# KyungMinJin/OTPose

Measured on AMD Instinct MI355X. Metric: frames/sec at 384x288, 5-frame window, batch 16; heatmap max-abs delta vs ref, higher is better.
Workload: dtype f32 storage+accumulate / f16x3 split products; 1 GPU; BASELINE configs[1]: batch 16 x 5-frame x 384x288, HRNet-W48 + DCN warp + ConvVideoTransformer, fp32 forward (eval), seeded synthetic weights; clips_per_gpu=16, parallelism=dp1, outputs_finite=True

## Files before the change

include/otpose_hip.h:

```cpp
#ifndef OTPOSE_HIP_H
#define OTPOSE_HIP_H

#include <stddef.h>

#ifdef __cplusplus
extern "C" {
#endif

#define OTP_OK 0
#define OTP_ERR_BAD_ARG (-1)
#define OTP_ERR_UNSUPPORTED (-2)
#define OTP_ERR_LAUNCH (-3)
#define OTP_ERR_WORKSPACE (-4)

#define OTP_DTYPE_F32 0
#define OTP_DTYPE_F16 1
#define OTP_DTYPE_BF16 2
#define OTP_DTYPE_F64 3
#define OTP_DTYPE_I64 4

#define OTP_ACT_NONE 0
#define OTP_ACT_RELU 1
#define OTP_ACT_GELU 2

// ... 160 lines not shown
                          size_t workspace_bytes, int B, int Cin, int J, int H, int W, const int* dilations, int ND, float alpha,
                          void* stream);

int otp_glue_total(const void* rough, void* total, void* squeezed, void* inter, void* flow_in, const void* pe,
                   int B, int J, int HW, void* stream);
int otp_glue_stack(const void* rough, const void* margin, const void* squeezed, const void* inter,
                   const void* ctx, const void* pe1, const void* pe2, void* x1, void* x2, void* prev_b,
                   int B, int J, int HW, void* stream);

int otp_glue_total_n(const void* rough, void* total, void* squeezed, void* inter, void* flow_in, const void* pe,
                     int B, int J, int HW, int F, void* stream);
int otp_glue_stack_n(const void* rough, const void* margin, const void* squeezed, const void* inter,
                     const void* ctx, const void* pe1, const void* pe2, void* x1, void* x2, void* prev_b,
                     int B, int J, int HW, int F, void* stream);

int otp_ln_channel(const void* x, const void* gamma, const void* beta, void* y, void* pool,
                   int B, int C, int T, float eps, void* stream);
int otp_dwconv_ln3(const void* x, const void* dwq, const void* dwk, const void* dwv,
                   const void* gq, const void* bq, const void* gk, const void* bk, const void* gv, const void* bv,
                   void* q, void* k, void* v, int B, int C, int T, int stride, float eps, void* stream);
size_t otp_chan_attn_workspace(int B, int C, int T, int n_head);
int otp_chan_attn(const void* q, const void* k, const void* v, void* out, void* workspace, size_t workspace_bytes,
                  int B, int C, int T, int n_head, float scale, void* stream);
int otp_upsample_linear(const void* x, void* out, int B, int C, int T, int f, int out_ctot, int out_coff, void* stream);

int otp_mlp_fused_supported(int C, int HID, int T);
size_t otp_mlp_fused_weight_bytes(int C, int HID);
int otp_mlp_fused_pack(const void* w1, const void* b1, const void* w2, void* packed, int C, int HID, void* stream);
int otp_mlp_fused(const void* x, const void* packed, const void* scale, const void* shift, const void* res, void* out,
                  int B, int C, int HID, int T, void* stream);
int otp_ln_mlp_fused(const void* y, const void* ln_gamma, const void* ln_beta, float ln_eps, const void* packed,
                     const void* scale, const void* shift, void* out, int B, int C, int HID, int T, void* stream);

int otp_dense_x3_supported(int C, int T);
size_t otp_dense_x3_weight_bytes(int C);
int otp_dense_x3_pack(const void* w, const void* scale, const void* shift, void* packed, int C, void* stream);
int otp_dense_x3(const void* const* x, const void* const* packed, const void* const* res, void* const* out, int nprob, int B,
                 int C, int T, void* stream);
int otp_dense_x3_pack_bf16p(const void* w, const void* scale, const void* shift, void* packed, int C, void* stream);
int otp_dense_x3_bf16p(const void* const* x, const void* const* packed, const void* const* res, void* const* out, int nprob, int B,
                 int C, int T, void* stream);
int otp_qkv_front_x3(const void* x, const void* table, const void* packed_q, const void* packed_k, const void* packed_v,
                     void* q, void* k, void* v, int B, int C, int T, float eps, void* stream);

int otp_stem_conv_x3_supported(int B, int F, int H, int W, int Cout);
size_t otp_stem_conv_x3_weight_bytes(int Cout);
int otp_stem_conv_x3_pack(const void* w, const void* scale, const void* shift, void* packed, int Cout, void* stream);
int otp_stem_conv_x3(const void* in, const void* packed, void* out, int B, int F, int H, int W, int Cout, void* stream);

int otp_pointwise_x3_supported(int Cin, int Cout, int T);
size_t otp_pointwise_x3_weight_bytes(int Cin, int Cout);
int otp_pointwise_x3_pack(const void* w, const void* scale, const void* shift, void* packed, int Cin, int Cout, void* stream);
int otp_pointwise_x3(const void* x, const void* packed, const void* res, void* out, int B, int Cin, int Cout, int T, int x_ctot,
                     int x_coff, int res_ctot, int res_coff, int out_ctot, int out_coff, int relu, void* stream);
int otp_pointwise_x3_s8_supported(int Cin, int Cout, int T);
size_t otp_pointwise_x3_s8_weight_bytes(int Cin, int Cout);
int otp_pointwise_x3_s8_pack(const void* w, const void* scale, const void* shift, void* packed, int Cin, int Cout, void* stream);
int otp_pointwise_x3_s8(const void* x, const void* packed, void* out_s8, int B, int Cin, int Cout, int T, int x_ctot, int x_coff,
                        int relu, void* stream);
int otp_pointwise_x3_s8_res(const void* x, const void* packed, const void* res, void* out_s8, int B, int Cin, int Cout, int T,
                            int x_ctot, int x_coff, int r_ctot, int r_coff, int relu, void* stream);
int otp_pointwise_x3_pair_supported(int Cin, int Cmid, int Cout2, int T);
size_t otp_pointwise_x3_pair_weight_bytes(int Cin, int Cmid, int Cout2);
int otp_pointwise_x3_pair_pack(const void* w1, const void* scale1, const void* shift1, const void* w2, const void* scale2,
                               const void* shift2, void* packed, int Cin, int Cmid, int Cout2, void* stream);
int otp_pointwise_x3_pair(const void* x, const void* packed, const void* res, void* out, void* out_s8, int B, int Cin, int Cmid,
                          int Cout2, int T, int x_ctot, int x_coff, int res_ctot, int res_coff, int out_ctot, int out_coff,
                          int relu1, int relu2, void* stream);

int otp_mlp_x3_supported(int C, int HID, int T);
size_t otp_mlp_x3_weight_bytes(int C, int HID);
int otp_mlp_x3_pack(const void* w1, const void* b1, const void* w2, void* packed, int C, int HID, void* stream);
int otp_mlp_x3(const void* x, const void* packed, const void* scale, const void* shift, const void* res, void* out, int B,
               int C, int HID, int T, void* stream);
int otp_ln_mlp_x3(const void* y, const void* ln_gamma, const void* ln_beta, float ln_eps, const void* packed,
                  const void* scale, const void* shift, void* out, int B, int C, int HID, int T, void* stream);

int otp_flow_block_supported(int C, int hidden, int T);
size_t otp_flow_front_param_floats(int C);
size_t otp_flow_back_param_floats(int C, int hidden);
int otp_flow_front(const void* x, const void* params, void* q, void* k, void* v, int B, int C, int T, float eps, void* stream);
int otp_flow_back(const void* x, const void* att, const void* params, void* out, int B, int C, int hidden, int T, float eps,
                  void* stream);

int otp_dense_cc_supported(int C, int T);
size_t otp_dense_cc_weight_bytes(int C);
int otp_dense_cc_pack(const void* w, const void* scale, const void* shift, void* packed, int C, void* stream);
int otp_dense_cc(const void* const* x, const void* const* packed, const void* const* res, void* const* out, int nprob,
                 int B, int C, int T, void* stream);

size_t otp_qkv_front_table_bytes(int C);
int otp_qkv_front_pack_table(const void* dwq, const void* dwk, const void* dwv, const void* gq, const void* bq,
                             const void* gk, const void* bk, const void* gv, const void* bv, void* table, int C,
                             void* stream);
int otp_qkv_front(const void* x, const void* table, const void* packed_q, const void* packed_k, const void* packed_v,
                  void* q, void* k, void* v, int B, int C, int T, float eps, void* stream);

int otp_upsample_add(const void* low, const void* res, void* out, int N, int C, int Hl, int Wl, int f, int relu,
                     int low_ctot, int low_coff, int res_ctot, int res_coff, int out_ctot, int out_coff, void* stream);
int otp_upsample_add_multi(const void* const* lows, const int* factors, int nlow, const void* res, void* out, int N, int C,
                           int Hh, int Wh, int relu, int res_ctot, int res_coff, int out_ctot, int out_coff, void* stream);

int otp_chan_attn_set_split(int on);
int otp_chan_attn_splits(int BH, int T);
int otp_chan_attn_scores(const void* a, const void* b, void* slabs, int BH, int hs, int T, void* stream);
int otp_chan_attn_apply(const void* v, const void* M, void* out, int BH, int hs, int T, void* stream);
int otp_chan_attn_scores_bf16p(const void* a, const void* b, void* slabs, int BH, int hs, int T, void* stream);
int otp_chan_attn_apply_bf16p(const void* v, const void* M, void* out, int BH, int hs, int T, void* stream);
int otp_transpose_scale(const void* in, void* out, int batches, int R, int Cc, float scale, void* stream);
int otp_softmax_backward(const void* slabs, const void* P, void* dS, void* dST, void* PT, int BH, int hs, int NS,
                         void* stream);
int otp_ln_channel_backward(const void* x, const void* grad_y, const void* gamma, void* grad_x, void* dy_xhat, int B, int C,
                            int T, float eps, void* stream);
size_t otp_ln_channel_backward_workspace(int B, int C, int T);
int otp_ln_channel_backward_params(const void* x, const void* grad_y, const void* gamma, void* grad_x, void* grad_gamma,
                                   void* grad_beta, void* workspace, size_t workspace_bytes, int B, int C, int T, float eps,
                                   void* stream);
int otp_dwconv3_forward(const void* x, const void* w, void* y, int B, int C, int T, int stride, void* stream);
int otp_dwconv3_backward(const void* x, const void* w, const void* grad_y, void* grad_x, void* grad_w, int B, int C, int T,
                         int stride, void* stream);
int otp_gelu_forward(const void* x, void* y, size_t n, void* stream);
int otp_gelu_backward(const void* x, const void* grad_y, void* grad_x, size_t n, void* stream);
int otp_maxpool3s2_forward(const void* x, void* y, int rows, int T, void* stream);
int otp_maxpool3s2_backward(const void* x, const void* grad_y, void* grad_x, int rows, int T, void* stream);
int otp_upsample_linear_backward(const void* grad_out, void* grad_x, int B, int C, int T, int f, int out_ctot, int out_coff,
                                 void* stream);

int otp_upsample_add_backward(const void* grad_out, const void* out_relu, void* grad_res, void* grad_low, int planes, int Hl,
                              int Wl, int f, void* stream);

int otp_axpby(const void* x, void* y, float alpha, float beta, size_t n, void* stream);

int otp_heatmap_decode(const void* heatmaps, void* preds, void* maxvals, const void* center, const void* scale,
                       int N, int J, int H, int W, int refine, void* stream);

int otp_heatmap_flip_decode(const void* heatmaps, const int* perm, void* merged, void* preds, void* maxvals,
                            const void* center, const void* scale, int B, int J, int H, int W, int shift, void* stream);
int otp_clip_mirror_pair(const void* x, void* out, int B, int C, int H, int W, void* stream);

int otp_pck_accuracy(const void* pred_coords, const void* target_coords, void* acc, void* cnt, int N, int J, int H, int W,
                     float thr, void* stream);

size_t otp_grad_sumsq_scratch(void);
int otp_grad_sumsq(const void* grad, size_t n, void* acc_f64, void* stream);
int otp_adamw_step(void* param, const void* grad, void* exp_avg, void* exp_avg_sq, size_t n, float lr, float beta1,
                   float beta2, float eps, float weight_decay, int step, const void* gradnorm_sq_f64, float max_norm,
                   void* stream);
int otp_sgd_step(void* param, const void* grad, void* momentum_buf, size_t n, float lr, float momentum, float dampening,
                 float weight_decay, int nesterov, int first_step, const void* gradnorm_sq_f64, float max_norm, void* stream);

int otp_ema_update(void* ema, const void* src, size_t n, float decay, float one_minus_decay, void* stream);
size_t otp_ema_job_bytes(void);
int otp_ema_job(void* ema, const void* src, size_t count, int dtype, const void* prev_job_host, void* job_host);
int otp_ema_update_table(const void* jobs_device, int n_jobs, float decay, float one_minus_decay, void* stream);

int otp_frames_u8_to_clip(const void* frames_u8, void* out, int B, int F, int H, int W, float mean_r, float mean_g,
                          float mean_b, float std_r, float std_g, float std_b, void* stream);

int otp_crop_clips_u8(const void* pool_u8, int S, int Hp, int Wp, const void* frame_idx, const void* M, const void* flip,
                      void* out, int B, int F, int H, int W, float mean_r, float mean_g, float mean_b, float std_r,
                      float std_g, float std_b, void* stream);
int otp_crop_clips_blur_u8(const void* pool_u8, int S, int Hp, int Wp, const void* frame_idx, const void* M,
                           const void* flip, void* out, int B, int F, int H, int W, float mean_r, float mean_g,
                           float mean_b, float std_r, float std_g, float std_b, const void* blur, const void* blur_on,
                           void* stream);
int otp_crop_clips_pair_u8(const void* pool_u8, int S, int Hp, int Wp, const void* frame_idx, const void* M, void* out,
// ... 122 lines not shown
```

otpose_amd/csrc/flowenc.hip:

```cpp
#include "common.h"

namespace {

template <int C>
__device__ __forceinline__ void fe_layer_norm(float (&v)[C], const float* __restrict__ g, const float* __restrict__ b, float eps) {
    float s = 0.f;
#pragma unroll
    for (int c = 0; c < C; ++c) s += v[c];
    const float mu = s * (1.f / C);
    float q = 0.f;
#pragma unroll
    for (int c = 0; c < C; ++c) {
        v[c] -= mu;
        q += v[c] * v[c];
    }
    const float rs = 1.f / sqrtf(q * (1.f / C) + eps);
#pragma unroll
    for (int c = 0; c < C; ++c) v[c] = v[c] * rs * g[c] + b[c];
}

template <int C>
constexpr int fe_front_floats() { return 2 * C + 3 * (3 * C + 2 * C + C * C + C); }
template <int C>
constexpr int fe_back_floats(int H) { return C * C + C + 2 * C + H * C + H + H * C + C; }

template <int C>
__global__ __launch_bounds__(192) void flow_front_kernel(const float* __restrict__ x, const float* __restrict__ prm,
                                                         float* __restrict__ q, float* __restrict__ k, float* __restrict__ v,
                                                         int T, float eps) {
    const int t = blockIdx.x * 64 + (threadIdx.x & 63);
    const int br = __builtin_amdgcn_readfirstlane(threadIdx.x >> 6);
    if (t >= T) return;
    const size_t base = (size_t)blockIdx.y * C * T + t;
    float n[3][C];
#pragma unroll
    for (int s = 0; s < 3; ++s) {
        const int tt = t - 1 + s;
        const bool ok = tt >= 0 && tt < T;
#pragma unroll
        for (int c = 0; c < C; ++c) n[s][c] = ok ? x[base + (size_t)c * T + (s - 1)] : 0.f;
        fe_layer_norm<C>(n[s], prm, prm + C, eps);
        if (!ok) {
#pragma unroll
            for (int c = 0; c < C; ++c) n[s][c] = 0.f;
        }
    }
    float* out = br == 0 ? q : (br == 1 ? k : v);
    const float* p = prm + 2 * C + br * (3 * C + 2 * C + C * C + C);
    float d[C];
#pragma unroll
    for (int c = 0; c < C; ++c) d[c] = p[c * 3] * n[0][c] + p[c * 3 + 1] * n[1][c] + p[c * 3 + 2] * n[2][c];
    fe_layer_norm<C>(d, p + 3 * C, p + 4 * C, eps);
    const float* W = p + 5 * C;
    const float* bias = W + C * C;
#pragma unroll
    for (int o = 0; o < C; ++o) {
        float a = bias[o];
#pragma unroll
        for (int c = 0; c < C; ++c) a = fmaf(W[o * C + c], d[c], a);
        out[base + (size_t)o * T] = a;
    }
}

template <int C>
__global__ __launch_bounds__(256) void flow_back_kernel(const float* __restrict__ x, const float* __restrict__ att,
                                                        const float* __restrict__ prm, float* __restrict__ out, int H, int T,
                                                        float eps) {
    __shared__ float part[3][C][64];
    const int lane = threadIdx.x & 63;
    const int wave = __builtin_amdgcn_readfirstlane(threadIdx.x >> 6);
    const int t = blockIdx.x * 64 + lane;
    const bool live = t < T;
    const size_t base = (size_t)blockIdx.y * C * T + (live ? t : 0);
    float a[C], y[C];
#pragma unroll
    for (int c = 0; c < C; ++c) {
        a[c] = att[base + (size_t)c * T];
        y[c] = x[base + (size_t)c * T];
    }
    const float* Wp = prm;
    const float* bp = Wp + C * C;
#pragma unroll
    for (int o = 0; o < C; ++o) {
        float s = bp[o];
#pragma unroll
        for (int c = 0; c < C; ++c) s = fmaf(Wp[o * C + c], a[c], s);
        y[o] += s;
    }
    float nn[C];
#pragma unroll
    for (int c = 0; c < C; ++c) nn[c] = y[c];
    fe_layer_norm<C>(nn, bp + C, bp + 2 * C, eps);
    const float* W1 = bp + 3 * C;
    const float* b1 = W1 + (size_t)H * C;
    const float* W2t = b1 + H;
    const float* b2 = W2t + (size_t)H * C;
    float acc[C];
#pragma unroll
    for (int o = 0; o < C; ++o) acc[o] = 0.f;
#pragma unroll 2
    for (int m = wave; m < H; m += 4) {
        float h = b1[m];
#pragma unroll
        for (int c = 0; c < C; ++c) h = fmaf(W1[m * C + c], nn[c], h);
        h = otp_gelu_erf(h);
#pragma unroll
        for (int o = 0; o < C; ++o) acc[o] = fmaf(W2t[m * C + o], h, acc[o]);
    }
    if (wave > 0) {
#pragma unroll
        for (int o = 0; o < C; ++o) part[wave - 1][o][lane] = acc[o];
    }
    __syncthreads();
    if (wave == 0 && live) {
#pragma unroll
        for (int o = 0; o < C; ++o)
            out[base + (size_t)o * T] = y[o] + b2[o] + ((acc[o] + part[0][o][lane]) + (part[1][o][lane] + part[2][o][lane]));
    }
}

}

extern "C" int otp_flow_block_supported(int C, int hidden, int T) { return (C == 17 && hidden > 0 && T > 0) ? 1 : 0; }

extern "C" size_t otp_flow_front_param_floats(int C) { return C == 17 ? (size_t)fe_front_floats<17>() : 0; }

extern "C" size_t otp_flow_back_param_floats(int C, int hidden) {
    return (C == 17 && hidden > 0) ? (size_t)fe_back_floats<17>(hidden) : 0;
}

extern "C" int otp_flow_front(const void* x, const void* params, void* q, void* k, void* v, int B, int C, int T, float eps,
                              void* stream) {
    if (!x || !params || !q || !k || !v || B <= 0 || T <= 0) return OTP_ERR_BAD_ARG;
    if (C != 17) return OTP_ERR_UNSUPPORTED;
    hipLaunchKernelGGL(flow_front_kernel<17>, dim3(otp_ceil_div(T, 64), B), dim3(192), 0, static_cast<hipStream_t>(stream),
                       static_cast<const float*>(x), static_cast<const float*>(params), static_cast<float*>(q),
                       static_cast<float*>(k), static_cast<float*>(v), T, eps);
    return otp_launch_status();
}

extern "C" int otp_flow_back(const void* x, const void* att, const void* params, void* out, int B, int C, int hidden, int T,
                             float eps, void* stream) {
    if (!x || !att || !params || !out || B <= 0 || T <= 0 || hidden <= 0) return OTP_ERR_BAD_ARG;
    if (C != 17) return OTP_ERR_UNSUPPORTED;
    hipLaunchKernelGGL(flow_back_kernel<17>, dim3(otp_ceil_div(T, 64), B), dim3(256), 0, static_cast<hipStream_t>(stream),
                       static_cast<const float*>(x), static_cast<const float*>(att), static_cast<const float*>(params),
                       static_cast<float*>(out), hidden, T, eps);
    return otp_launch_status();
}
```

otpose_amd/engine.py:

```python
from __future__ import annotations

import ctypes
import dataclasses
import os
import sys
import warnings
from typing import Callable, List, Optional, Tuple

import torch

from . import hip, ops
from .ops import ACT_GELU, ACT_NONE, ACT_RELU, View

def _pair(v):
    return (int(v), int(v)) if isinstance(v, int) else (int(v[0]), int(v[1]))


def plain_conv(cv, k, stride=1, pad="same", dil=1, groups=1, bias=False, cin=None, cout=None) -> bool:
    if pad == "same":
        pad = (dil or 1) * (k // 2)
    return (cv.kernel_size == (k, k) and (stride is None or cv.stride == (stride, stride))
            and (pad is None or tuple(cv.padding) == (pad, pad)) and (dil is None or tuple(cv.dilation) == (dil, dil))
            and (groups is None or cv.groups == groups) and (bias is None or (cv.bias is not None) == bias)
            and (cin is None or cv.in_channels == cin) and (cout is None or cv.out_channels == cout))
# ... 10 lines not shown
    use_small_conv: bool = True
    use_fused_mlp: bool = True
    fuse_shortcut: bool = True
    fuse_upsample: bool = True
    use_dense_cc: bool = True
    use_qkv_front: bool = True
    use_pointx: bool = True
    pointx_fuse: bool = True
    pointx_any: bool = False
    multi_stream: bool = True
    f32_tail: int = 0
    h16_tail: bool = True
    range_check: str = "defer"
    s8_residual: bool = True
    s8_lazy_nchw: bool = True
    s8_stride2: bool = True
    t1_s8: bool = True
    l1_s8: bool = True
    l1_pair: bool = True
    stem_x3: bool = True
    chain_modules: bool = True
    up_any_width: bool = True
    conv_log: bool = False
    poison: Optional[Tuple[int, int]] = None
    te_serial: bool = False

    @classmethod
    def from_env(cls) -> "Routes":
        env = os.environ.get
        on = lambda name: env("OTPOSE_" + name, "1") != "0"
        x3 = env("OTPOSE_CONV_MATH", "x3") != "f32"
        poison = env("OTPOSE_POISON")
        return cls(use_graph=on("HIP_GRAPH"), use_winograd=on("WINOGRAD"), use_x3=x3, use_dcn_fused=x3 and on("DCN_FUSED"),
                   use_s8=x3 and on("S8"), use_flow_fused=on("FLOW_FUSED"), use_small_conv=on("SMALL_CONV"),
                   use_fused_mlp=on("FUSED_MLP"), fuse_shortcut=on("FUSE_SHORTCUT"), fuse_upsample=on("FUSE_UPSAMPLE"),
                   use_dense_cc=on("DENSE_CC"), use_qkv_front=on("QKV_FRONT"), use_pointx=x3 and on("POINTX"),
                   pointx_fuse=on("POINTX_FUSE"), pointx_any=env("OTPOSE_POINTX_ANY", "0") == "1", multi_stream=on("STREAMS"),
                   f32_tail=int(env("OTPOSE_F32_TAIL", "0")) if x3 else 0, h16_tail=on("H16_TAIL"),
                   range_check=env("OTPOSE_RANGE_CHECK", "defer"), s8_residual=on("S8_RESIDUAL"), s8_lazy_nchw=on("S8_LAZY_NCHW"),
                   s8_stride2=on("S8_STRIDE2"), t1_s8=on("T1_S8"), l1_s8=on("L1_S8"), l1_pair=on("L1_PAIR"), stem_x3=on("STEM_X3"),
                   chain_modules=on("CHAIN_MODULES"), up_any_width=on("UP_ANY_WIDTH"), conv_log=bool(env("OTPOSE_CONV_LOG")),
                   poison=tuple(int(v) for v in poison.split(":")) if poison else None, te_serial=env("OTPOSE_TE_SERIAL") == "1")

    @property
    def lazy_nchw(self) -> bool:
        return self.s8_residual and self.s8_lazy_nchw


class Aux:
    __slots__ = ("s8", "c4", "nchw_needed")

    def __init__(self, s8=None, c4=None, nchw_needed=False):
        self.s8, self.c4, self.nchw_needed = s8, c4, nchw_needed


class InferenceEngine:
    h16 = False

    def __init__(self, model, batch: int, device, use_graph: bool | None = None, stream_set: int = 0, inp=None, margin=None):
        routes = Routes.from_env()
        self._init(device, routes, routes.use_graph if use_graph is None else use_graph, stream_set)
        self.B = batch
        self.model = model
        cfg = model.cfg
        self.J = model.num_joints
        self.F = getattr(model, "window_frames", 5)
        self.W_img, self.H_img = cfg.MODEL.IMAGE_SIZE
        self.h, self.w = model.pe_h, model.pe_w
        self._given = (inp, margin)
        self.param_version = self._param_version()
        with torch.no_grad():
            self._build()

    def _init(self, device, routes: Routes, use_graph: bool, stream_set: int = 0):
        device = torch.device(device)
        if device.type != "cuda" or not torch.cuda.is_available():
            raise RuntimeError("otpose_amd.OTPose runs on an MI355X through libotpose_hip.so; "
                               f"got device '{device}' (there is no CPU or PyTorch-op fallback)")
        self.lib, self.dev, self.routes = hip.lib(), device, routes
        self.model, self.B, self.inp, self.margin = None, 0, None, None
        self.ops: List[Callable] = []
        self._pair_s8 = {}
        self.l1_pairs = 0
        self._aux = {}
        self._keep = []
        self._bufs = []
        self._stream = None
        self.use_graph, self.graph = use_graph, None
        self._exact = False
        self._sid = 0
        self._side = hip.side_streams(device, 3, 4 * stream_set) if routes.multi_stream else []

    @classmethod
    def bare(cls, device, multi_stream=False):
        self = cls.__new__(cls)
        self._init(device, dataclasses.replace(Routes.from_env(), multi_stream=bool(multi_stream)), use_graph=False)
        return self

    use_x3 = property(lambda self: self.routes.use_x3)
    use_dcn_fused = property(lambda self: self.routes.use_dcn_fused)
    multi_stream = property(lambda self: self.routes.multi_stream)
    f32_tail = property(lambda self: self.routes.f32_tail)
    range_check = property(lambda self: self.routes.range_check)
    half_products = property(lambda self: self.h16 and self.routes.use_x3 and self.routes.h16_tail)

    @property
    def s8_here(self) -> bool:
        return self.routes.use_s8 and not self._exact

    @property
    def s2_here(self) -> bool:
        return self.routes.use_s8 and not self._exact and self.routes.s8_stride2

    def matches(self, x) -> bool:
        return (x.shape[0] == self.B and x.device == self.dev and tuple(x.shape[2:]) == (self.H_img, self.W_img)
                and self._param_version() == self.param_version)

    def matches_shape(self, b, c, h, w, dev) -> bool:
        return (b == self.B and dev == self.dev and (h, w) == (self.H_img, self.W_img) and c == 3 * self.F
                and self._param_version() == self.param_version)

    def _param_version(self):
        ts = getattr(self, "_tracked", None)
        if ts is None:
            ts = self._tracked = list(self.model.parameters()) + list(self.model.buffers())
        v = a = 0
        for t in ts:
            v += t._version
            a ^= t.data_ptr()
        return (len(ts), v, a)

    def new(self, *shape):
        t = torch.empty(shape, dtype=torch.float32, device=self.dev)
        rng = self.routes.poison
        if rng and rng[0] <= len(self._bufs) < rng[1]:
            t.fill_(float("nan"))
        self._bufs.append(t)
        return t

    def dev_param(self, t):
        t = t.detach().to(self.dev, torch.float32).contiguous()
        self._keep.append(t)
        return t

    winograd_pays = staticmethod(ops.winograd_pays)

    def _emit(self, fn):
        self.ops.append((fn, self._sid))

    def fork(self, sids):
        if not self.multi_stream:
            return
        sids = [s for s in sids if 0 < s <= len(self._side)]

        def run():
            main = torch.cuda.current_stream(self.dev)
            for s_ in sids:
                self._side[s_ - 1].wait_stream(main)
        self.ops.append((run, -1))

    def join(self, sids):
        if not self.multi_stream:
            return
        sids = [s for s in sids if 0 < s <= len(self._side)]

        def run():
# ... 478 lines not shown
                cont = (self.routes.chain_modules and nxt is not None and len(mod.fuse_layers) == nxt.num_branches
                        and mod.num_branches > 1)
                ys = module(s, mi, len(mods), mod, ys, fork_in, not cont)
        return ys

    def hrnet(self, net, x_in: View) -> View:
        c1 = net.conv1
        r = self.routes
        n_in, c_in, h_in, w_in = x_in.t.shape
        if (r.use_x3 and r.stem_x3 and x_in.coff == 0 and x_in.C == c_in and c_in == 3 * self.F and plain_conv(c1, 3, stride=2, cin=3)
                and ops.stem_conv_x3_supported(n_in, self.F, h_in, w_in, c1.out_channels)):
            sc, sh = self._bn_fold(net.bn1)
            pk = ops.pack_stem_conv_x3(self.dev_param(c1.weight), sc, sh)
            self._keep.append(pk)
            x = View(self.new(self.F * n_in, c1.out_channels, (h_in - 1) // 2 + 1, (w_in - 1) // 2 + 1))
            self.call(self.lib.otp_stem_conv_x3, "otp_stem_conv_x3", *ops.stem_conv_x3_args(x_in.t, pk, x.t, self.F, c1.out_channels))
        else:
            x = self.conv_bn(x_in, net.conv1, net.bn1, ACT_RELU, frame_split=self.B, cin=3)
        blocks = list(net.layer1)
        b0 = blocks[0]
        if (r.fuse_shortcut and b0.downsample is not None and plain_conv(b0.conv3, 1) and plain_conv(b0.downsample[0], 1)):
            n, _, h, w = x.t.shape
            c2 = net.conv2
            ho = (h + 2 * c2.padding[0] - c2.kernel_size[0]) // c2.stride[0] + 1
            wo = (w + 2 * c2.padding[0] - c2.kernel_size[0]) // c2.stride[0] + 1
            cx, cy = c2.out_channels, b0.conv2.out_channels
            cat = self.new(n, cx + cy, ho, wo)
            xin = self.conv_bn(x, c2, net.bn2, ACT_RELU, out=View(cat, 0, cx))
            if self.conv1_conv2_s8(xin, b0.conv1, b0.bn1, b0.conv2, b0.bn2, out=View(cat, cx, cy)) is None:
                y = self.conv_bn(xin, b0.conv1, b0.bn1, ACT_RELU)
                self.conv_bn(y, b0.conv2, b0.bn2, ACT_RELU, out=View(cat, cx, cy))

            def fold(conv, bn):
                sc, sh = self._bn_fold(bn)
                return self.dev_param(conv.weight) * sc[:, None, None, None], sh
            wd, shd = fold(b0.downsample[0], b0.downsample[1])
            w3, sh3 = fold(b0.conv3, b0.bn3)
            cout = b0.conv3.out_channels
            wcat, ones, shcat = torch.cat([wd, w3], 1), torch.ones(cout, device=self.dev), shd + sh3
            x = self.pointx_pair(View(cat), wcat, ones, shcat, None, blocks[1]) if len(blocks) > 1 else None
            if x is None:
                x = self.conv(View(cat), wcat, View(self.new(n, cout, ho, wo)), scale=ones, shift=shcat, act=ACT_RELU)
            blocks = blocks[1:]
        else:
            x = self.conv_bn(x, net.conv2, net.bn2, ACT_RELU)
        for bi, blk in enumerate(blocks):
            x = self.bottleneck(blk, x, s8_only=self.s2_here and r.t1_s8 and bi == len(blocks) - 1,
                                nxt=blocks[bi + 1] if bi + 1 < len(blocks) else None)

        def t1_s8(s):
            return s == 2 and self.s8_here and r.t1_s8

        def before_fork(s, ys):
            if (s >= 3 or t1_s8(s)) and self.s2_here:
                self.s8_image(ys[-1], want_c4=s >= 3 and not r.s8_residual)

        def width_change(s, x, tr):
            y = self.conv_bn_s8(x, tr[0], tr[1], ACT_RELU) if t1_s8(s) else None
            return y if y is not None else self.conv_bn(x, tr[0], tr[1], ACT_RELU)

        def new_branch(s, z, tr):
            zs = self.s2_chain_s8([(step[0], step[1], True) for step in tr], z, ACT_RELU) if (s >= 3 or t1_s8(s)) else None
            if zs is not None:
                return zs
            for step in tr:
                z = self.conv_bn(z, step[0], step[1], ACT_RELU)
            return z

        def module(s, mi, n_mods, mod, xs, fork_in, join_out):
            self._exact = s == 4 and mi >= n_mods - r.f32_tail
            return self.hr_module(mod, xs, fork_in, join_out)
        ys = self.hr_stages(net, x, width_change, new_branch, module, before_fork)
        fl = net.final_layer
        rough = View(self.new(self.F * self.B, self.J, self.h, self.w))
        self._exact = r.f32_tail > 0
        out = self.conv(ys[0], fl.weight, rough, 1, fl.padding[0], 1, bias=fl.bias)
        self._exact = False
        return out

    def v3(self, t3):
        b, c, t = t3.shape
        return View(t3.view(b, c, 1, t))

    def tblock(self, blk, x, stride):
        B, C, T = x.shape
        To = T if stride == 1 else (T + 2 - 3) // 2 + 1
        L = self.lib
        a = blk.attn
        r = self.routes
        if r.use_flow_fused and stride == 1 and ops.flow_block_supported(blk, C, T):
            fp, bp = ops.pack_flow_front(blk, self.dev), ops.pack_flow_back(blk, self.dev)
            self._keep += [fp, bp]
            q, k, v, att, out = (self.new(B, C, T) for _ in range(5))
            self.call(L.otp_flow_front, "otp_flow_front", *ops.flow_front_args(x, fp, q, k, v, blk.ln1.eps))
            self.chan_attn(q, k, v, att, a)
            self.call(L.otp_flow_back, "otp_flow_back", *ops.flow_back_args(x, att, bp, out, blk.mlp[0].out_channels, blk.ln2.eps))
            return out
        ln1 = self.new(B, C, T)
        skip = self.new(B, C, To) if stride > 1 else None
        p = self.dev_param
        self.call(L.otp_ln_channel, "otp_ln_channel", hip.ptr(x), hip.ptr(p(blk.ln1.weight)), hip.ptr(p(blk.ln1.bias)),
                  hip.ptr(ln1), hip.ptr(skip), B, C, T, blk.ln1.eps)
        q, k, v = self.new(B, C, To), self.new(B, C, To), self.new(B, C, To)
        dx3 = r.use_dense_cc and r.use_x3 and ops.dense_x3_supported(C, To)
        dense = dx3 or (r.use_dense_cc and ops.dense_cc_supported(C, To))
        if dense:
            packs = [ops.pack_dense_cc(m.weight.to(self.dev), None, m.bias.to(self.dev), x3=dx3)
                     for m in (a.query, a.key, a.value)]
        if dense and stride == 1 and r.use_qkv_front:
            table = ops.pack_qkv_table(*[p(t) for t in (a.query_conv.weight, a.key_conv.weight, a.value_conv.weight,
                                                         a.query_norm.weight, a.query_norm.bias, a.key_norm.weight,
                                                         a.key_norm.bias, a.value_norm.weight, a.value_norm.bias)])
            self._keep += [table, *packs]
            self.call((L.otp_qkv_front_h1 if self.half_products else L.otp_qkv_front_x3) if dx3 else L.otp_qkv_front, "otp_qkv_front",
                      *ops.qkv_front_args(ln1, table, packs, (q, k, v), a.query_norm.eps))
        else:
            qn, kn, vn = self.new(B, C, To), self.new(B, C, To), self.new(B, C, To)
            self.call(L.otp_dwconv_ln3, "otp_dwconv_ln3", hip.ptr(ln1), hip.ptr(p(a.query_conv.weight)),
                      hip.ptr(p(a.key_conv.weight)), hip.ptr(p(a.value_conv.weight)),
                      hip.ptr(p(a.query_norm.weight)), hip.ptr(p(a.query_norm.bias)),
                      hip.ptr(p(a.key_norm.weight)), hip.ptr(p(a.key_norm.bias)),
                      hip.ptr(p(a.value_norm.weight)), hip.ptr(p(a.value_norm.bias)),
                      hip.ptr(qn), hip.ptr(kn), hip.ptr(vn), B, C, T, stride, a.query_norm.eps)
            if dense:
                self.dense((qn, kn, vn), packs, None, (q, k, v), B, C, To)
            else:
                self.conv(self.v3(qn), a.query.weight, self.v3(q), bias=a.query.bias)
                self.conv(self.v3(kn), a.key.weight, self.v3(k), bias=a.key.bias)
                self.conv(self.v3(vn), a.value.weight, self.v3(v), bias=a.value.bias)
        att = self.new(B, C, To)
        self.chan_attn(q, k, v, att, a)
        sa = blk.drop_path_attn.scale.detach().reshape(-1)
        y = self.new(B, C, To)
        if dense:
            sad = sa.to(self.dev, torch.float32)
            pk = ops.pack_dense_cc(a.proj.weight.to(self.dev), sad, a.proj.bias.detach().to(self.dev) * sad,
                                   x3=r.use_x3 and ops.dense_x3_supported(C, To))
            self.dense((att,), [pk], (skip if stride > 1 else x,), (y,), B, C, To)
        else:
            self.conv(self.v3(att), a.proj.weight, self.v3(y), scale=sa,
                      shift=a.proj.bias.detach() * sa.to(a.proj.bias.device), res=self.v3(skip if stride > 1 else x))
        sm = blk.drop_path_mlp.scale.detach().reshape(-1)
        out = self.new(B, C, To)
        hid = blk.mlp[0].out_channels
        mlp_x3 = r.use_fused_mlp and r.use_x3 and ops.mlp_x3_supported(C, hid, To)
        if mlp_x3 or (r.use_fused_mlp and ops.mlp_fused_supported(C, hid, To)):
            dev = lambda t: t.detach().to(self.dev, torch.float32)
            w1, b1, w2 = dev(blk.mlp[0].weight), dev(blk.mlp[0].bias), dev(blk.mlp[3].weight)
            packed = ops.pack_mlp_x3_weights(w1, b1, w2, half=self.half_products) if mlp_x3 else ops.pack_mlp_weights(w1, b1, w2)
            scd = dev(sm).contiguous()
            shd = (dev(blk.mlp[3].bias) * scd).contiguous()
            self._keep += [packed, scd, shd]
            fn, name = ((L.otp_ln_mlp_h1 if self.half_products else L.otp_ln_mlp_x3, "otp_ln_mlp_x3") if mlp_x3
                        else (L.otp_ln_mlp_fused, "otp_ln_mlp_fused"))
            self.call(fn, name, *ops.ln_mlp_args(y, p(blk.ln2.weight), p(blk.ln2.bias), blk.ln2.eps, packed, scd, shd, out, hid))
            return out
        ln2 = self.new(B, C, To)
        self.call(L.otp_ln_channel, "otp_ln_channel", hip.ptr(y), hip.ptr(p(blk.ln2.weight)), hip.ptr(p(blk.ln2.bias)),
                  hip.ptr(ln2), None, B, C, To, blk.ln2.eps)
        hdn = self.new(B, 4 * C, To)
        self.conv(self.v3(ln2), blk.mlp[0].weight, self.v3(hdn), bias=blk.mlp[0].bias, act=ACT_GELU)
        self.conv(self.v3(hdn), blk.mlp[3].weight, self.v3(out), scale=sm,
                  shift=blk.mlp[3].bias.detach() * sm.to(blk.mlp[3].bias.device), res=self.v3(y))
        return out

    def chan_attn(self, q, k, v, att, a):
        B, C, T = q.shape
        nbytes = self.lib.otp_chan_attn_workspace(B, C, T, a.n_head)
        ws = self.new(max(nbytes // 4, 1))
        self.call(self.lib.otp_chan_attn, "otp_chan_attn", *ops.chan_attn_args(q, k, v, att, ws, nbytes, a.n_head, a.scale))

    def conv_transformer(self, ct, x, stacked):
        _, C, T = x.shape
        L = self.lib
        for blk in ct.stem:
            x = self.tblock(blk, x, 1)
        self.call(L.otp_upsample_linear, "otp_upsample_linear", *ops.upsample_linear_args(x, stacked, 1, 0))
        for i, blk in enumerate(ct.branch):
            x = self.tblock(blk, x, 2)
            f = 2 ** (i + 1)
            if x.shape[2] * f != T:
                raise RuntimeError("heat-map size must make every pyramid level divide evenly (T % 4 == 0)")
            self.call(L.otp_upsample_linear, "otp_upsample_linear", *ops.upsample_linear_args(x, stacked, f, (i + 1) * C))

    def rsb_block(self, blk, x: View) -> View:
        n, _, h, w = x.t.shape
        bc = blk.branch_ch
        cbr = lambda m, inp, out, act, in2=None, res=None: self.conv(
            inp, m.conv.weight, out, 1, m.conv.padding[0], 1, bn=m.bn, bias=m.conv.bias, act=act, in2=in2, res=res)
        t = self.new(n, 4 * bc, h, w)
        cat = self.new(n, 4 * bc, h, w)
        cbr(blk.conv_bn_relu1, x, View(t), ACT_RELU)
        s = [View(t, i * bc, bc) for i in range(4)]
        tmp = lambda: View(self.new(n, bc, h, w))
        par = self.multi_stream and self._sid == 0
        side = (lambda: (self.fork((1,)), self.on_stream(1))) if par else (lambda: None)
        main = (lambda: self.on_stream(0)) if par else (lambda: None)
        o11 = cbr(blk.conv_bn_relu2_1_1, s[0], View(cat, 0, bc), ACT_RELU)
        o21 = cbr(blk.conv_bn_relu2_2_1, s[1], tmp(), ACT_RELU, in2=o11)
        side()
        o22 = cbr(blk.conv_bn_relu2_2_2, o21, View(cat, bc, bc), ACT_RELU)
        main()
        o31 = cbr(blk.conv_bn_relu2_3_1, s[2], tmp(), ACT_RELU, in2=o21)
        side()
        o32 = cbr(blk.conv_bn_relu2_3_2, o31, tmp(), ACT_RELU, in2=o22)
        main()
        o41 = cbr(blk.conv_bn_relu2_4_1, s[3], tmp(), ACT_RELU, in2=o31)
        if par:
            self.join((1,))
        o42 = cbr(blk.conv_bn_relu2_4_2, o41, tmp(), ACT_RELU, in2=o32)
        if par:
            self.on_stream(1)
        o33 = cbr(blk.conv_bn_relu2_3_3, o32, View(cat, 2 * bc, bc), ACT_RELU)
        if par:
            self.on_stream(0)
            self.join((1,))
        o43 = cbr(blk.conv_bn_relu2_4_3, o42, tmp(), ACT_RELU, in2=o33)
        cbr(blk.conv_bn_relu2_4_4, o43, View(cat, 3 * bc, bc), ACT_RELU)
        res = x
        if blk.downsample is not None:
            res = cbr(blk.downsample, x, View(self.new(n, blk.conv_bn_relu3.conv.out_channels, h, w)), ACT_NONE)
        out = View(self.new(n, blk.conv_bn_relu3.conv.out_channels, h, w))
        return cbr(blk.conv_bn_relu3, View(cat), out, ACT_RELU, res=res)

    def rsb_chain(self, chain, x: View) -> View:
        for blk in chain.layers:
            x = self.rsb_block(blk, x)
        return x

    def _build(self):
        m, B, J, h, w = self.model, self.B, self.J, self.h, self.w
        L, T = self.lib, self.h * self.w
        self.inp = self._given[0] if self._given[0] is not None else self.new(B, 3 * self.F, self.H_img, self.W_img)
        self.margin = self._given[1] if self._given[1] is not None else self.new(B, self.F - 1)
        assert tuple(self.inp.shape) == (B, 3 * self.F, self.H_img, self.W_img) and self.inp.is_contiguous()
        rough = self.hrnet(m.rough_pose_estimation_net, View(self.inp)).t
        self.hr_end = len(self.ops)

        total, squeezed, inter = self.new(B, J, h, w), self.new(B, J, h, w), self.new(B, J, h, w)
        flow_in = self.new(B, J, T)
        pe_f = self.dev_param(m.flow_encoder.pos_embd[0, :, :T])
        self.call(L.otp_glue_total_n, "otp_glue_total", hip.ptr(rough), hip.ptr(total), hip.ptr(squeezed), hip.ptr(inter),
                  hip.ptr(flow_in), hip.ptr(pe_f), B, J, T, self.F)
        ctx = self.new(B, J, T)
        self.fork((2,))
        self.on_stream(2)
        def_h = self.rsb_chain(m.def_fuse, View(total))
        self.on_stream(0)
        self.conv_transformer(m.flow_encoder, flow_in, ctx)
        D = m.num_frames * J
        x1, x2, prev_b = self.new(B, D, T), self.new(B, D, T), self.new(B, J, h, w)
        pe1 = self.dev_param(m.temporal_encoder1.pos_embd[0, :, :T])
        pe2 = self.dev_param(m.temporal_encoder2.pos_embd[0, :, :T])
        self.call(L.otp_glue_stack_n, "otp_glue_stack", hip.ptr(rough), hip.ptr(self.margin), hip.ptr(squeezed),
                  hip.ptr(inter), hip.ptr(ctx), hip.ptr(pe1), hip.ptr(pe2), hip.ptr(x1), hip.ptr(x2), hip.ptr(prev_b),
                  B, J, T, self.F)
        levels = m.scale_arch[-1] + 1
        cs_ = levels * D
        cpad = (-cs_) % 32 if (self.use_x3 and m.final_layer1.kernel_size == (1, 1)) else 0
# ... 141 lines not shown
```

otpose_amd/ops.py:

```python
from __future__ import annotations

import ctypes
import math
import os

import torch
from torch.autograd import Function

from . import hip
from .augment import FLIP_PAIRS

_K = hip.CONSTANTS
_DTYPE_F32 = _K["OTP_DTYPE_F32"]


def _require_gpu(*tensors):
    for t in tensors:
        if t is not None and not t.is_cuda:
            raise NotImplementedError("otpose_amd operators run on the GPU only (no CPU path)")


def _check_f32(*tensors):
    for t in tensors:
        if t is not None and t.dtype != torch.float32:
# ... 1425 lines not shown
    return out


def _joints_mse(o, g, w, topk, ohkm, effective_num_joints, with_grad):
    _require_gpu(o, g)
    b, j = o.shape[:2]
    hw = o[0, 0].numel()
    o, g = o.contiguous(), g.contiguous()
    wv = None if w is None else w.reshape(b, j).contiguous().float()
    L = hip.lib()
    nbytes = L.otp_loss_workspace(b, j)
    ws = torch.empty(nbytes // 4, dtype=torch.float32, device=o.device)
    res = torch.empty(3, dtype=torch.float32, device=o.device)
    go = torch.empty_like(o) if with_grad else None
    hip.check(L.otp_loss_joints_mse(hip.ptr(o), hip.ptr(g), hip.ptr(wv), hip.ptr(res), hip.ptr(go), hip.ptr(ws), nbytes,
                                    b, j, hw, topk, int(ohkm), int(effective_num_joints or 0), hip.stream_of(o)),
              "otp_loss_joints_mse")
    return res, go


def joints_ohkm_mse_loss(output, target, target_weight=None, effective_num_joints=None, topk=8, with_grad=False):
    res, go = _joints_mse(output, target, target_weight, topk, True, effective_num_joints, with_grad)
    out = {"ohkm_loss": res[0], "mse_loss": res[1], "final_loss": res[2]}
    if with_grad:
        out["grad_output"] = go
    return out


def joint_mse_loss(output, target, target_weight=None, effective_num_joints=None, with_grad=False):
    res, go = _joints_mse(output, target, target_weight, 1, False, effective_num_joints, with_grad)
    return (res[2], go) if with_grad else res[2]


def flow_block_supported(blk, c, t) -> bool:
    a = blk.attn
    try:
        eps = {float(m.eps) for m in (blk.ln1, a.query_norm, a.key_norm, a.value_norm)}
        has_bias = all(m.bias is not None for m in (a.query, a.key, a.value, a.proj, blk.mlp[0], blk.mlp[3]))
        dw_ok = all(tuple(m.weight.shape) == (c, 1, 3) and m.bias is None for m in (a.query_conv, a.key_conv, a.value_conv))
    except AttributeError:
        return False
    return (len(eps) == 1 and has_bias and dw_ok
            and bool(hip.lib().otp_flow_block_supported(int(c), int(blk.mlp[0].out_channels), int(t))))


def pack_flow_front(blk, device):
    a = blk.attn
    f = lambda t: t.detach().to(device, torch.float32).reshape(-1)
    parts = [f(blk.ln1.weight), f(blk.ln1.bias)]
    for conv, norm, proj in ((a.query_conv, a.query_norm, a.query), (a.key_conv, a.key_norm, a.key),
                             (a.value_conv, a.value_norm, a.value)):
        parts += [f(conv.weight), f(norm.weight), f(norm.bias), f(proj.weight), f(proj.bias)]
    prm = torch.cat(parts).contiguous()
    c = blk.ln1.weight.numel()
    assert prm.numel() == hip.lib().otp_flow_front_param_floats(c), (prm.numel(), c)
    return prm


def pack_flow_back(blk, device):
    a = blk.attn
    d = lambda t: t.detach().to(device, torch.float32)
    c = blk.ln1.weight.numel()
    hid = blk.mlp[0].out_channels
    sa, sm = d(blk.drop_path_attn.scale).reshape(-1), d(blk.drop_path_mlp.scale).reshape(-1)
    wp = d(a.proj.weight).reshape(c, c) * sa[:, None]
    w2 = d(blk.mlp[3].weight).reshape(c, hid) * sm[:, None]
    parts = [wp.reshape(-1), d(a.proj.bias) * sa, d(blk.ln2.weight).reshape(-1), d(blk.ln2.bias).reshape(-1),
             d(blk.mlp[0].weight).reshape(-1), d(blk.mlp[0].bias), w2.t().contiguous().reshape(-1), d(blk.mlp[3].bias) * sm]
    prm = torch.cat(parts).contiguous()
    assert prm.numel() == hip.lib().otp_flow_back_param_floats(c, hid), (prm.numel(), c, hid)
    return prm


def flow_front_args(x, prm, q, k, v, eps):
    b, c, t = x.shape
    return (hip.ptr(x), hip.ptr(prm), hip.ptr(q), hip.ptr(k), hip.ptr(v), b, c, t, float(eps))


def flow_back_args(x, att, prm, out, hidden, eps):
    b, c, t = x.shape
    return (hip.ptr(x), hip.ptr(att), hip.ptr(prm), hip.ptr(out), b, c, int(hidden), t, float(eps))


def flow_front(x, prm, eps=1e-5):
    _require_gpu(x, prm)
    _check_f32(x)
    x = x.contiguous()
    q, k, v = torch.empty_like(x), torch.empty_like(x), torch.empty_like(x)
    _launch(hip.lib().otp_flow_front, "otp_flow_front", flow_front_args(x, prm, q, k, v, eps), x)
    return q, k, v


def flow_back(x, att, prm, hidden, eps=1e-5):
    _require_gpu(x, att, prm)
    _check_f32(x)
    x, att = x.contiguous(), att.contiguous()
    out = torch.empty_like(x)
    _launch(hip.lib().otp_flow_back, "otp_flow_back", flow_back_args(x, att, prm, out, hidden, eps), x)
    return out


class H8:

    __slots__ = ("t", "N", "C", "H", "W", "gtot", "goff")

    def __init__(self, t, n, c, h, w, gtot=None, goff=0):
        assert c % 8 == 0
        self.t, self.N, self.C, self.H, self.W = t, n, c, h, w
        self.gtot, self.goff = (c // 8 if gtot is None else gtot), goff
        assert 0 <= self.goff and self.goff + c // 8 <= self.gtot

    def slice(self, coff, c):
        assert coff % 8 == 0 and c % 8 == 0 and coff + c <= self.C
        return H8(self.t, self.N, c, self.H, self.W, self.gtot, self.goff + coff // 8)


def h8_empty(n, c, h, w, device):
    nbytes = hip.lib().otp_h8_bytes(n, c, h, w)
    if not nbytes:
        raise ValueError(f"H8 images need a channel count that is a multiple of 8, got {c}")
    return H8(torch.empty(nbytes // 4, dtype=torch.int32, device=device), n, c, h, w)


def h8_pack(x, out: H8 = None, stream=None):
    iv = x if isinstance(x, View) else View(x.contiguous())
    _require_gpu(iv.t)
    n, _, h, w = iv.t.shape
    out = h8_empty(n, iv.C, h, w, iv.t.device) if out is None else out
    hip.check(hip.lib().otp_h8_pack(hip.ptr(iv.t), hip.ptr(out.t), n, iv.C, h, w, iv.ctot, iv.coff, out.gtot, out.goff,
                                    stream if stream is not None else hip.stream_of(iv.t)), "otp_h8_pack")
    return out


def h8_unpack(img: H8, stream=None):
    out = torch.empty(img.N, img.C, img.H, img.W, dtype=torch.float32, device=img.t.device)
    hip.check(hip.lib().otp_h8_unpack(hip.ptr(img.t), hip.ptr(out), img.N, img.C, img.H, img.W, img.gtot, img.goff,
                                      stream if stream is not None else hip.stream_of(img.t)), "otp_h8_unpack")
    return out


def h16_weight_exponent(weight, scale=None) -> int:
    w = weight.detach()
    m = w.abs().reshape(w.shape[0], -1).amax(dim=1)
    if scale is not None:
        m = m * scale.detach().abs().to(m.device, m.dtype)
    m = float(m.max())
    if not (m > 0.0 and math.isfinite(m)):
        return 0
    return max(-40, min(40, 14 - math.frexp(m)[1]))


def h16_conv_desc(x: H8, cout, stride, act=ACT_NONE, out: H8 = None, res: H8 = None, k=0):
    d = hip.H16ConvDesc()
    d.N, d.Cin, d.H, d.W, d.Cout, d.stride, d.act = x.N, x.C, x.H, x.W, cout, stride, act
    d.in_gtot, d.in_goff = x.gtot, x.goff
    d.out_gtot, d.out_goff = (out.gtot, out.goff) if out is not None else (0, 0)
    d.res_gtot, d.res_goff = (res.gtot, res.goff) if res is not None else (0, 0)
    d.out_scale = 2.0 ** -k
    return d


def h16_conv_supported(desc) -> bool:
    return bool(hip.lib().otp_h16_conv3x3_supported(desc))


def pack_h16_conv_weight(weight, scale=None, k=0):
    _require_gpu(weight)
    w = _f32(weight)
    cout, cin, kh, kw = w.shape
    assert (kh, kw) == (3, 3)
    L = hip.lib()
    packed = _image(L.otp_h16_conv3x3_weight_bytes(cout, cin), torch.int32, w.device,
                    RuntimeError, f"otp_h16_conv3x3: unsupported widths {cin} -> {cout}", zero=True)
    sc = _f32(scale, w.device)
    hip.check(L.otp_h16_conv3x3_pack_weight(hip.ptr(w), hip.ptr(sc), hip.ptr(packed), cout, cin, float(2.0 ** k), hip.stream_of(w)),
              "otp_h16_conv3x3_pack_weight")
    return packed


def h16_conv3x3_args(x: H8, wpacked, shift, out: H8, desc, res: H8 = None):
    return (_vp(x), hip.ptr(wpacked), hip.ptr(shift), _vp(res), _vp(out), desc)

# ... 225 lines not shown
```

Baseline: 3324 frames/s.

## Fuse flow-block back half with next block's QKV front via halo tile

```diff
diff --git a/include/otpose_hip.h b/include/otpose_hip.h
--- a/include/otpose_hip.h
+++ b/include/otpose_hip.h
@@ -266,6 +266,8 @@
 int otp_flow_front(const void* x, const void* params, void* q, void* k, void* v, int B, int C, int T, float eps, void* stream);
 int otp_flow_back(const void* x, const void* att, const void* params, void* out, int B, int C, int hidden, int T, float eps,
                   void* stream);
+int otp_flow_back_front(const void* x, const void* att, const void* back_params, const void* front_params, void* out, void* q,
+                        void* k, void* v, int B, int C, int hidden, int T, float eps_back, float eps_front, void* stream);
 
 int otp_dense_cc_supported(int C, int T);
 size_t otp_dense_cc_weight_bytes(int C);
diff --git a/otpose_amd/csrc/flowenc.hip b/otpose_amd/csrc/flowenc.hip
--- a/otpose_amd/csrc/flowenc.hip
+++ b/otpose_amd/csrc/flowenc.hip
@@ -23,6 +23,83 @@
 constexpr int fe_front_floats() { return 2 * C + 3 * (3 * C + 2 * C + C * C + C); }
 template <int C>
 constexpr int fe_back_floats(int H) { return C * C + C + 2 * C + H * C + H + H * C + C; }
+
+template <int C, class Ld, class Ok, class St>
+__device__ __forceinline__ void fe_front_token(const float* __restrict__ prm, int br, float eps, Ld ld, Ok ok_at, St st) {
+    float n[3][C];
+#pragma unroll
+    for (int s = 0; s < 3; ++s) {
+        const bool ok = ok_at(s);
+#pragma unroll
+        for (int c = 0; c < C; ++c) n[s][c] = ok ? ld(c, s) : 0.f;
+        fe_layer_norm<C>(n[s], prm, prm + C, eps);
+        if (!ok) {
+#pragma unroll
+            for (int c = 0; c < C; ++c) n[s][c] = 0.f;
+        }
+    }
+    const float* p = prm + 2 * C + br * (3 * C + 2 * C + C * C + C);
+    float d[C];
+#pragma unroll
+    for (int c = 0; c < C; ++c) d[c] = p[c * 3] * n[0][c] + p[c * 3 + 1] * n[1][c] + p[c * 3 + 2] * n[2][c];
+    fe_layer_norm<C>(d, p + 3 * C, p + 4 * C, eps);
+    const float* W = p + 5 * C;
+    const float* bias = W + C * C;
+#pragma unroll
+    for (int o = 0; o < C; ++o) {
+        float a = bias[o];
+#pragma unroll
+        for (int c = 0; c < C; ++c) a = fmaf(W[o * C + c], d[c], a);
+        st(o, a);
+    }
+}
+
+template <int C>
+__device__ __forceinline__ const float* fe_back_token(const float* __restrict__ x, const float* __restrict__ att,
+                                                      const float* __restrict__ prm, size_t base, int wave, int H, int T,
+                                                      float eps, float (&y)[C], float (&acc)[C]) {
+    float a[C];
+#pragma unroll
+    for (int c = 0; c < C; ++c) {
+        a[c] = att[base + (size_t)c * T];
+        y[c] = x[base + (size_t)c * T];
+    }
+    const float* Wp = prm;
+    const float* bp = Wp + C * C;
+#pragma unroll
+    for (int o = 0; o < C; ++o) {
+        float s = bp[o];
+#pragma unroll
+        for (int c = 0; c < C; ++c) s = fmaf(Wp[o * C + c], a[c], s);
+        y[o] += s;
+    }
+    float nn[C];
+#pragma unroll
+    for (int c = 0; c < C; ++c) nn[c] = y[c];
+    fe_layer_norm<C>(nn, bp + C, bp + 2 * C, eps);
+    const float* W1 = bp + 3 * C;
+    const float* b1 = W1 + (size_t)H * C;
+    const float* W2t = b1 + H;
+    const float* b2 = W2t + (size_t)H * C;
+#pragma unroll
+    for (int o = 0; o < C; ++o) acc[o] = 0.f;
+#pragma unroll 2
+    for (int m = wave; m < H; m += 4) {
+        float h = b1[m];
+#pragma unroll
+        for (int c = 0; c < C; ++c) h = fmaf(W1[m * C + c], nn[c], h);
+        h = otp_gelu_erf(h);
+#pragma unroll
+        for (int o = 0; o < C; ++o) acc[o] = fmaf(W2t[m * C + o], h, acc[o]);
+    }
+    return b2;
+}
+
+template <int C>
+__device__ __forceinline__ float fe_back_join(const float (&y)[C], const float* __restrict__ b2, const float (&acc)[C],
+                                              const float (&part)[3][C][64], int lane, int o) {
+    return y[o] + b2[o] + ((acc[o] + part[0][o][lane]) + (part[1][o][lane] + part[2][o][lane]));
+}
 
 template <int C>
 __global__ __launch_bounds__(192) void flow_front_kernel(const float* __restrict__ x, const float* __restrict__ prm,
@@ -32,34 +109,10 @@
     const int br = __builtin_amdgcn_readfirstlane(threadIdx.x >> 6);
     if (t >= T) return;
     const size_t base = (size_t)blockIdx.y * C * T + t;
-    float n[3][C];
-#pragma unroll
-    for (int s = 0; s < 3; ++s) {
-        const int tt = t - 1 + s;
-        const bool ok = tt >= 0 && tt < T;
-#pragma unroll
-        for (int c = 0; c < C; ++c) n[s][c] = ok ? x[base + (size_t)c * T + (s - 1)] : 0.f;
-        fe_layer_norm<C>(n[s], prm, prm + C, eps);
-        if (!ok) {
-#pragma unroll
-            for (int c = 0; c < C; ++c) n[s][c] = 0.f;
-        }
-    }
     float* out = br == 0 ? q : (br == 1 ? k : v);
-    const float* p = prm + 2 * C + br * (3 * C + 2 * C + C * C + C);
-    float d[C];
-#pragma unroll
-    for (int c = 0; c < C; ++c) d[c] = p[c * 3] * n[0][c] + p[c * 3 + 1] * n[1][c] + p[c * 3 + 2] * n[2][c];
-    fe_layer_norm<C>(d, p + 3 * C, p + 4 * C, eps);
-    const float* W = p + 5 * C;
-    const float* bias = W + C * C;
-#pragma unroll
-    for (int o = 0; o < C; ++o) {
-        float a = bias[o];
-#pragma unroll
-        for (int c = 0; c < C; ++c) a = fmaf(W[o * C + c], d[c], a);
-        out[base + (size_t)o * T] = a;
-    }
+    fe_front_token<C>(
+        prm, br, eps, [&](int c, int s) { return x[base + (size_t)c * T + (s - 1)]; },
+        [&](int s) { return t - 1 + s >= 0 && t - 1 + s < T; }, [&](int o, float a) { out[base + (size_t)o * T] = a; });
 }
 
 template <int C>
@@ -72,41 +125,8 @@
     const int t = blockIdx.x * 64 + lane;
     const bool live = t < T;
     const size_t base = (size_t)blockIdx.y * C * T + (live ? t : 0);
-    float a[C], y[C];
-#pragma unroll
-    for (int c = 0; c < C; ++c) {
-        a[c] = att[base + (size_t)c * T];
-        y[c] = x[base + (size_t)c * T];
-    }
-    const float* Wp = prm;
-    const float* bp = Wp + C * C;
-#pragma unroll
-    for (int o = 0; o < C; ++o) {
-        float s = bp[o];
-#pragma unroll
-        for (int c = 0; c < C; ++c) s = fmaf(Wp[o * C + c], a[c], s);
-        y[o] += s;
-    }
-    float nn[C];
-#pragma unroll
-    for (int c = 0; c < C; ++c) nn[c] = y[c];
-    fe_layer_norm<C>(nn, bp + C, bp + 2 * C, eps);
-    const float* W1 = bp + 3 * C;
-    const float* b1 = W1 + (size_t)H * C;
-    const float* W2t = b1 + H;
-    const float* b2 = W2t + (size_t)H * C;
-    float acc[C];
-#pragma unroll
-    for (int o = 0; o < C; ++o) acc[o] = 0.f;
-#pragma unroll 2
-    for (int m = wave; m < H; m += 4) {
-        float h = b1[m];
-#pragma unroll
-        for (int c = 0; c < C; ++c) h = fmaf(W1[m * C + c], nn[c], h);
-        h = otp_gelu_erf(h);
-#pragma unroll
-        for (int o = 0; o < C; ++o) acc[o] = fmaf(W2t[m * C + o], h, acc[o]);
-    }
+    float y[C], acc[C];
+    const float* b2 = fe_back_token<C>(x, att, prm, base, wave, H, T, eps, y, acc);
     if (wave > 0) {
 #pragma unroll
         for (int o = 0; o < C; ++o) part[wave - 1][o][lane] = acc[o];
@@ -114,8 +134,47 @@
     __syncthreads();
     if (wave == 0 && live) {
 #pragma unroll
-        for (int o = 0; o < C; ++o)
-            out[base + (size_t)o * T] = y[o] + b2[o] + ((acc[o] + part[0][o][lane]) + (part[1][o][lane] + part[2][o][lane]));
+        for (int o = 0; o < C; ++o) out[base + (size_t)o * T] = fe_back_join<C>(y, b2, acc, part, lane, o);
+    }
+}
+
+constexpr int FE_PAIR_OWN = 62;
+template <int C>
+__global__ __launch_bounds__(256) void flow_pair_kernel(const float* __restrict__ x, const float* __restrict__ att,
+                                                        const float* __restrict__ bprm, const float* __restrict__ fprm,
+                                                        float* __restrict__ out, float* __restrict__ q, float* __restrict__ k,
+                                                        float* __restrict__ v, int H, int T, float eps_back, float eps_front) {
+    __shared__ float part[3][C][64];
+    __shared__ float tile[C][64];
+    const int lane = threadIdx.x & 63;
+    const int wave = __builtin_amdgcn_readfirstlane(threadIdx.x >> 6);
+    const int t = blockIdx.x * FE_PAIR_OWN - 1 + lane;
+    const bool live = t >= 0 && t < T;
+    const bool own = live && lane >= 1 && lane <= FE_PAIR_OWN;
+    const size_t base = (size_t)blockIdx.y * C * T + (live ? t : 0);
+    {
+        float y[C], acc[C];
+        const float* b2 = fe_back_token<C>(x, att, bprm, base, wave, H, T, eps_back, y, acc);
+        if (wave > 0) {
+#pragma unroll
+            for (int o = 0; o < C; ++o) part[wave - 1][o][lane] = acc[o];
+        }
+        __syncthreads();
+        if (wave == 0) {
+#pragma unroll
+            for (int o = 0; o < C; ++o) {
+                const float r = fe_back_join<C>(y, b2, acc, part, lane, o);
+                tile[o][lane] = r;
+                if (own) out[base + (size_t)o * T] = r;
+            }
+        }
+    }
+    __syncthreads();
+    if (wave < 3 && own) {
+        float* dst = wave == 0 ? q : (wave == 1 ? k : v);
+        fe_front_token<C>(
+            fprm, wave, eps_front, [&](int c, int s) { return tile[c][lane - 1 + s]; },
+            [&](int s) { return t - 1 + s >= 0 && t - 1 + s < T; }, [&](int o, float a) { dst[base + (size_t)o * T] = a; });
     }
 }
 
@@ -148,3 +207,17 @@
                        static_cast<float*>(out), hidden, T, eps);
     return otp_launch_status();
 }
+
+extern "C" int otp_flow_back_front(const void* x, const void* att, const void* back_params, const void* front_params, void* out,
+                                   void* q, void* k, void* v, int B, int C, int hidden, int T, float eps_back, float eps_front,
+                                   void* stream) {
+    if (!x || !att || !back_params || !front_params || !out || !q || !k || !v || B <= 0 || T <= 0 || hidden <= 0)
+        return OTP_ERR_BAD_ARG;
+    if (C != 17) return OTP_ERR_UNSUPPORTED;
+    hipLaunchKernelGGL(flow_pair_kernel<17>, dim3(otp_ceil_div(T, FE_PAIR_OWN), B), dim3(256), 0,
+                       static_cast<hipStream_t>(stream), static_cast<const float*>(x), static_cast<const float*>(att),
+                       static_cast<const float*>(back_params), static_cast<const float*>(front_params),
+                       static_cast<float*>(out), static_cast<float*>(q), static_cast<float*>(k), static_cast<float*>(v), hidden,
+                       T, eps_back, eps_front);
+    return otp_launch_status();
+}
diff --git a/otpose_amd/engine.py b/otpose_amd/engine.py
--- a/otpose_amd/engine.py
+++ b/otpose_amd/engine.py
@@ -116,6 +116,8 @@
         self.ops: List[Callable] = []
         self._pair_s8 = {}
         self.l1_pairs = 0
+        self.flow_pair = os.environ.get("OTPOSE_FLOW_PAIR", "1") != "0"
+        self.flow_pairs = 0
         self._aux = {}
         self._keep = []
         self._bufs = []
@@ -760,20 +762,41 @@
         b, c, t = t3.shape
         return View(t3.view(b, c, 1, t))
 
+    def flow_route(self, blk, C, T) -> bool:
+        return self.routes.use_flow_fused and ops.flow_block_supported(blk, C, T)
+
+    def flow_block(self, blk, x, qkv=None, nxt=None):
+        B, C, T = x.shape
+        L = self.lib
+        bp = ops.pack_flow_back(blk, self.dev)
+        self._keep.append(bp)
+        if qkv is None:
+            fp = ops.pack_flow_front(blk, self.dev)
+            self._keep.append(fp)
+            qkv = tuple(self.new(B, C, T) for _ in range(3))
+            self.call(L.otp_flow_front, "otp_flow_front", *ops.flow_front_args(x, fp, *qkv, blk.ln1.eps))
+        att, out = self.new(B, C, T), self.new(B, C, T)
+        self.chan_attn(*qkv, att, blk.attn)
+        hid = blk.mlp[0].out_channels
+        if nxt is None:
+            self.call(L.otp_flow_back, "otp_flow_back", *ops.flow_back_args(x, att, bp, out, hid, blk.ln2.eps))
+            return out, None
+        fpn = ops.pack_flow_front(nxt, self.dev)
+        self._keep.append(fpn)
+        nqkv = tuple(self.new(B, C, T) for _ in range(3))
+        self.flow_pairs += 1
+        self.call(L.otp_flow_back_front, "otp_flow_back_front",
+                  *ops.flow_back_front_args(x, att, bp, fpn, out, *nqkv, hid, blk.ln2.eps, nxt.ln1.eps))
+        return out, nqkv
+
     def tblock(self, blk, x, stride):
         B, C, T = x.shape
         To = T if stride == 1 else (T + 2 - 3) // 2 + 1
         L = self.lib
         a = blk.attn
         r = self.routes
-        if r.use_flow_fused and stride == 1 and ops.flow_block_supported(blk, C, T):
-            fp, bp = ops.pack_flow_front(blk, self.dev), ops.pack_flow_back(blk, self.dev)
-            self._keep += [fp, bp]
-            q, k, v, att, out = (self.new(B, C, T) for _ in range(5))
-            self.call(L.otp_flow_front, "otp_flow_front", *ops.flow_front_args(x, fp, q, k, v, blk.ln1.eps))
-            self.chan_attn(q, k, v, att, a)
-            self.call(L.otp_flow_back, "otp_flow_back", *ops.flow_back_args(x, att, bp, out, blk.mlp[0].out_channels, blk.ln2.eps))
-            return out
+        if stride == 1 and self.flow_route(blk, C, T):
+            return self.flow_block(blk, x)[0]
         ln1 = self.new(B, C, T)
         skip = self.new(B, C, To) if stride > 1 else None
         p = self.dev_param
@@ -851,8 +874,13 @@
     def conv_transformer(self, ct, x, stacked):
         _, C, T = x.shape
         L = self.lib
-        for blk in ct.stem:
-            x = self.tblock(blk, x, 1)
+        stem, qkv = list(ct.stem), None
+        for i, blk in enumerate(stem):
+            if not self.flow_route(blk, C, T):
+                x = self.tblock(blk, x, 1)
+                continue
+            nxt = stem[i + 1] if self.flow_pair and i + 1 < len(stem) and self.flow_route(stem[i + 1], C, T) else None
+            x, qkv = self.flow_block(blk, x, qkv, nxt)
         self.call(L.otp_upsample_linear, "otp_upsample_linear", *ops.upsample_linear_args(x, stacked, 1, 0))
         for i, blk in enumerate(ct.branch):
             x = self.tblock(blk, x, 2)
diff --git a/otpose_amd/ops.py b/otpose_amd/ops.py
--- a/otpose_amd/ops.py
+++ b/otpose_amd/ops.py
@@ -1531,6 +1531,12 @@
     return (hip.ptr(x), hip.ptr(att), hip.ptr(prm), hip.ptr(out), b, c, int(hidden), t, float(eps))
 
 
+def flow_back_front_args(x, att, bprm, fprm, out, q, k, v, hidden, eps_back, eps_front):
+    b, c, t = x.shape
+    return (hip.ptr(x), hip.ptr(att), hip.ptr(bprm), hip.ptr(fprm), hip.ptr(out), hip.ptr(q), hip.ptr(k), hip.ptr(v), b, c,
+            int(hidden), t, float(eps_back), float(eps_front))
+
+
 def flow_front(x, prm, eps=1e-5):
     _require_gpu(x, prm)
     _check_f32(x)
@@ -1547,6 +1553,16 @@
     out = torch.empty_like(x)
     _launch(hip.lib().otp_flow_back, "otp_flow_back", flow_back_args(x, att, prm, out, hidden, eps), x)
     return out
+
+
+def flow_back_front(x, att, bprm, fprm, hidden, eps_back=1e-5, eps_front=1e-5):
+    _require_gpu(x, att, bprm, fprm)
+    _check_f32(x)
+    x, att = x.contiguous(), att.contiguous()
+    out, q, k, v = (torch.empty_like(x) for _ in range(4))
+    _launch(hip.lib().otp_flow_back_front, "otp_flow_back_front",
+            flow_back_front_args(x, att, bprm, fprm, out, q, k, v, hidden, eps_back, eps_front), x)
+    return out, q, k, v
 
 
 class H8:
```

Result: no change. 3320 frames/s (-0.1%).
